# RalphAS/PeriodicSchurDecompositions.jl

Hardware: AMD Instinct MI355X
Metric: PSD sweeps/sec (pschur! n=1024 p=64 Float64, Hessenberg+Q+iteration, operands in HBM) (higher is better)
Workload: dtype f64

## Files before the change

### periodicschurdecompositions.jl_amd/csrc/psd_engine.cpp

```cpp
#include <atomic>
#include "psd_hess.h"
#include "psd_bhess.h"
#include "psd_hess2.h"
#include "psd_formq2.h"
#include "psd_real_qr.h"
#include "psd_apply2.h"
#include "psd_zhess.h"
#include "psd_zhess2.h"
#include "psd_zqz.h"
#include "psd_zord.h"
#include "psd_rord.h"
#include "psd_rgz.h"
#include "psd_zgz.h"
#include "psd_zgord.h"
#include "psd_grord.h"
#include "psd_rhessx.h"
#include "psd_check.h"
#include "psd_krylov.h"
#include "psd_evec.h"
#include "psd_gevec.h"
#include "psd_bevec.h"
#include "psd_zbevec.h"
#include "psd_bord.h"
#include "psd_zbqz.h"
// ... 190 lines not shown
        PSD_CHECK(psd_rt_malloc((void**)&tcnt, 2 * sizeof(int) * PSD_SLOTS * (size_t)(p + 8)));
        PSD_CHECK(psd_rt_malloc((void**)&ttr, 2 * sizeof(psd_tr) * PSD_SLOTS * (size_t)p * PSD_TR_CAP));
        PSD_CHECK(psd_rt_malloc((void**)&tgl, sizeof(psd_rglobal)));
        PSD_CHECK(psd_rt_malloc((void**)&tslotw, sizeof(int) * (8 * PSD_SLOTS + PSD_PLAN_INTS)));
        tcap_p = p;
        return 0;
    }
    void trelease() {
        if (tcst) psd_rt_free(tcst);
        if (tshift) psd_rt_free(tshift);
        if (tdesc) psd_rt_free(tdesc);
        if (tcnt) psd_rt_free(tcnt);
        if (ttr) psd_rt_free(ttr);
        if (tgl) psd_rt_free(tgl);
        if (tslotw) psd_rt_free(tslotw);
        tcst = nullptr; tshift = nullptr; tdesc = nullptr; tcnt = nullptr; ttr = nullptr;
        tgl = nullptr; tslotw = nullptr;
        tcap_p = 0;
    }
    double* fqT = nullptr;
    size_t fqT_doubles = 0;
    int formq_blocked = 1;
#ifndef PSD_HOSTSIM
    hipGraphExec_t hess_exec = nullptr;
    int hess_graph_n = 0, hess_graph_p = 0;
    double* h2ring = nullptr;
    int h2ring_n = 0;
    double* zh2ring = nullptr;
    int zh2ring_n = 0;
    std::vector<hipEvent_t> h2ev;
    int hess_async = -1;
    int hess_lookahead = 1;
    int hess_xcd = 1;
    int hess_fit = 15;
#endif
    int shard_rank = 0, shard_world = 1;
    int batch_group = 0;
    int bh_nmax = PSD_BH_NMAX;
    int zb_nmax = PSD_ZB_NMAX;
    int bev_nmax = PSD_BEV_NMAX;
    int bord_nmax = PSD_BORD_NMAX;
    int bord_w = 0;
    void slice(int p, int& lo, int& hi) const {
        const int base = p / shard_world, rem = p % shard_world;
        lo = shard_rank * base + (shard_rank < rem ? shard_rank : rem);
        hi = lo + base + (shard_rank < rem ? 1 : 0);
    }
    int train_stop = 1;
    int train_wdiv = 0;
    int train_long = 256;
    int band_helper = 1;
    int zstream = 3;
    int zcdefer = 0;
    int redge = 0, cedge = 0;
    int rdefer = 1;
    int cdefer = 1;
    int overlap = 3;
    int far_grid = 0;
    bool counted = false;
    bool pipe_ok = false;
#ifndef PSD_HOSTSIM
    hipStream_t stream2 = nullptr;
    hipStream_t stream3 = nullptr;
    hipStream_t stream4 = nullptr;
    int hess_pipe_depth = 3;
    int hess_pipe = 1;
// ... 341 lines not shown
};
#endif

namespace {

void fill_bytes(psd_stats* s, int n, int p, int wantT, int wantZ, const std::vector<int>& log) {
    if (!s) return;
    double b = 0.0;
    const double E = 8.0;
    for (size_t q = 0; q + 2 < log.size(); q += 3) {
        if (log[q] != 0) continue;
        const double w = log[q + 2] - log[q + 1] + 1;
        if (!wantT) b += 2 * E * p * w * w + (wantZ ? 2 * E * p * w * n : 0.0);
        else b += 2 * E * p * w * (wantZ ? (2.0 * n + 1) : (n + 1.0));
    }
    s->bytes_sweeps = b;
}

static inline bool psd_pipe_form(const psd_ctx* c) {
#ifndef PSD_HOSTSIM
    if (!c->stream4 || c->hess_pipe == 0) return false;
    return c->hess_pipe == 2 || c->shard_world > 1 || c->pipe_ok;
#else
    (void)c;
    return false;
#endif
}

#ifndef PSD_HOSTSIM

struct h2_diag {
    psd_ctx* c;
    long long* t = nullptr;
    static constexpr size_t words = 1024 * 8 + 1024 * 4;
    h2_diag(psd_ctx* c_, psd_hess2_args& ha) : c(c_) {
        ha.fault = -1;
        if (const char* e = psd_env_diag("PSD_H2_FAULT")) ha.fault = atoi(e);
        ha.trace = nullptr;
        ha.trace_hi = 0x7fffffff;
        const char* e = psd_env_diag("PSD_H2_TRACE");
        if (!e) return;
        if (atoi(e) > 1) ha.trace_hi = atoi(e);
        if (psd_rt_malloc((void**)&t, words * sizeof(long long)) != 0) t = nullptr;
        else if (psd_rt_memset(t, 0, words * sizeof(long long), c->stream) == 0) ha.trace = t;
    }
    ~h2_diag() {
        if (!t) return;
        std::vector<long long> h(words);
        (void)psd_rt_sync(c->stream);
        (void)hipMemcpy(h.data(), t, sizeof(long long) * h.size(), hipMemcpyDeviceToHost);
        double acc[8] = {0};
        int cnt = 0;
        double per = 0;
        for (int q = 1; q < 1023; ++q) {
            const long long* a = &h[(size_t)q * 8];
            const long long* pr = &h[(size_t)(q - 1) * 8];
            if (a[0] == 0 || a[6] == 0 || pr[0] == 0 || a[0] < pr[0]) continue;
            for (int k = 1; k <= 6; ++k) acc[k] += (double)(a[k] - a[k - 1]);
            per += (double)(a[0] - pr[0]);
            ++cnt;
        }
        if (cnt) fprintf(stderr, "psd hess2 trace (last %d links, block 2, us): link period %.2f | ring loads %.2f | norm reduce %.2f | larfg %.2f | v to LDS + publish %.2f | gemv %.2f | finish %.2f\n", cnt, per / cnt / 100.0, acc[1] / cnt / 100.0, acc[2] / cnt / 100.0, acc[3] / cnt / 100.0, acc[4] / cnt / 100.0, acc[5] / cnt / 100.0, acc[6] / cnt / 100.0);
        const long long* bk = &h[1024 * 8];
        long long t0 = 0;
        for (int q = 0; q < 1024; ++q)
            if (bk[4 * q] && (!t0 || bk[4 * q] < t0)) t0 = bk[4 * q];
        if (t0) {
            fprintf(stderr, "psd hess2 trace, one link, per block (start, end in us after the first start):");
            for (int q = 0; q < 1024; ++q)
                if (bk[4 * q] && (q < 12 || q % 16 == 0)) fprintf(stderr, " b%d %.2f-%.2f", q, (bk[4 * q] - t0) / 100.0, (bk[4 * q + 1] - t0) / 100.0);
            double lastend = 0, maxstart = 0;
            for (int q = 0; q < 1024; ++q)
                if (bk[4 * q]) {
                    if ((bk[4 * q + 1] - t0) / 100.0 > lastend) lastend = (bk[4 * q + 1] - t0) / 100.0;
                    if ((bk[4 * q] - t0) / 100.0 > maxstart) maxstart = (bk[4 * q] - t0) / 100.0;
                }
            fprintf(stderr, " | last start %.2f last end %.2f\n", maxstart, lastend);
        }
        psd_rt_free(t);
    }
};
struct h2_no_diag {
    h2_no_diag(psd_ctx*, psd_zhess2_args&) {}
};

template <typename T> struct h2_type;
template <> struct h2_type<double> {
    typedef psd_hess2_args args;
    typedef h2_diag diag;
    static constexpr int NT = PSD_H2_NT, ROWS = PSD_H2_ROWS;
    static constexpr int CR_LARGE = 8;
    static constexpr int PIPE_NMAX = 2048;
    static constexpr bool FIT = true;
    template <int NKB> static constexpr int CPW = (NKB <= 16) ? 4 : 1;
    template <int NK, int CR>
    static void link(int grid, size_t lds, hipStream_t s, const args& ha, int n, int i, int j, int nC, int nT) {
        hipLaunchKernelGGL((psd_hess2_link<NK, CR>), dim3(grid), dim3(NT), lds, s, ha, n, i, j, nC, nT);
    }
    template <int NK, int CPW_>
    static void bulk(int gridx, int K, size_t lds, hipStream_t s, const args& ha, int n, int idx0, int nT) {
        hipLaunchKernelGGL((psd_hess2_bulk<NK, CPW_>), dim3(gridx, K), dim3(NT), lds, s, ha, n, idx0, nT);
    }
    static double*& ring(psd_ctx* c) { return c->h2ring; }
    static int& ring_n(psd_ctx* c) { return c->h2ring_n; }
    static size_t slot_doubles(int n) { return psd_h2_slot_doubles(n); }
    static int pipe(const psd_ctx* c, int n, args& ha) {
        ha.pipe = 2;
        if (n > 512 && n <= 1024) ha.xcd = 0;
        return (c->hess_pipe_depth >= 3 && c->stream2 && n <= 1024) ? 3 : 2;
    }
};
template <> struct h2_type<psd_z> {
    typedef psd_zhess2_args args;
    typedef h2_no_diag diag;
    static constexpr int NT = PSD_ZH2_NT, ROWS = PSD_ZH2_ROWS;
    static constexpr int CR_LARGE = 4;
    static constexpr int PIPE_NMAX = 1024;
    static constexpr bool FIT = false;
    template <int NKB> static constexpr int CPW = 1;
    template <int NK, int CR>
    static void link(int grid, size_t lds, hipStream_t s, const args& ha, int n, int i, int j, int nC, int nT) {
        hipLaunchKernelGGL((psd_zhess2_link<NK, CR>), dim3(grid), dim3(NT), lds, s, ha, n, i, j, nC, nT);
    }
    template <int NK, int>
    static void bulk(int gridx, int K, size_t lds, hipStream_t s, const args& ha, int n, int idx0, int nT) {
        hipLaunchKernelGGL((psd_zhess2_bulk<NK>), dim3(gridx, K), dim3(NT), lds, s, ha, n, idx0, nT);
    }
    static double*& ring(psd_ctx* c) { return c->zh2ring; }
    static int& ring_n(psd_ctx* c) { return c->zh2ring_n; }
    static size_t slot_doubles(int n) { return psd_zh2_slot_doubles(n); }
    static int pipe(const psd_ctx*, int, args& ha) {
        ha.pipe = 1;
        return 2;
    }
};

template <typename T> size_t h2_lds(int n) { return ((size_t)n + 8 + 2 * h2_type<T>::NT + 64) * sizeof(T); }
template <typename T, int CR> struct h2_grid {
    static constexpr int RPL = 128 / (int)sizeof(T), G = 8 * RPL / CR;
    int nC, nT;
    h2_grid(int n, int xcd) {
        const int nc = (n + CR - 1) / CR;
        nC = ((xcd && CR < RPL) ? (nc + G - 1) / G * G : nc) + 1;
        nT = (n + h2_type<T>::ROWS - 1) / h2_type<T>::ROWS;
    }
};

template <typename T, int NKB, int CR> struct h2_launcher {
    typedef h2_type<T> Tr;
    typedef typename Tr::args args;
    static constexpr int CPW = Tr::template CPW<NKB>;
    const h2_grid<T, CR> g;
    const size_t lds;
    const int n, p, GS;
    const int fit;
    const args& ha;
    h2_launcher(psd_ctx* c, int n_, int p_, const args& ha_)
        : g(n_, ha_.xcd), lds(h2_lds<T>(n_)), n(n_), p(p_), GS((ha_.xcd && CR < g.RPL) ? g.RPL / CR : 0), fit(Tr::FIT ? c->hess_fit : 0), ha(ha_) {}
    void link(hipStream_t s, int i, int j, bool fused) const {
        psd_h2_geom q{NKB, g.nC, fused ? g.nT : 0, fused ? (n + 3) / 4 : 0};
        if constexpr (Tr::FIT) {
            if (fit) {
                const psd_h2_geom f = psd_h2_fit_chain(n, p, (i - 1) * p + (p - j), CR, GS, fused);
                if (fit & 1) q.nC = f.nC;
                if (fit & 2) q.NK = f.NK;
                if (fit & 4) q.nT = f.nT, q.nB = f.nB;
                const int grid = q.nC + q.nT + q.nB;
                switch (q.NK) {
                    case 4: if constexpr (NKB > 4) return Tr::template link<4, CR>(grid, lds, s, ha, n, i, j, q.nC, q.nT); break;
                    case 8: if constexpr (NKB > 8) return Tr::template link<8, CR>(grid, lds, s, ha, n, i, j, q.nC, q.nT); break;
                    case 16: if constexpr (NKB > 16) return Tr::template link<16, CR>(grid, lds, s, ha, n, i, j, q.nC, q.nT); break;
                    default: break;
                }
            }
        }
        Tr::template link<NKB, CR>(q.nC + q.nT + q.nB, lds, s, ha, n, i, j, q.nC, q.nT);
    }
    void bulk(hipStream_t s, int idx0, int K) const {
        psd_h2_geom q{NKB, 0, g.nT, (n + 3) / 4};
        if constexpr (Tr::FIT) {
            if (fit) {
                psd_h2_geom f = q;
                psd_h2_fit_panel(n, p, idx0, K, 4 * CPW, f);
                if (fit & 4) q.nT = f.nT, q.nB = f.nB;
                if (fit & 8) q.NK = f.NK;
                const int gx = q.nT + q.nB > 0 ? q.nT + q.nB : 1;
                switch (q.NK) {
                    case 4: if constexpr (NKB > 4) return Tr::template bulk<4, CPW>(gx, K, lds, s, ha, n, idx0, q.nT); break;
                    case 8: if constexpr (NKB > 8) return Tr::template bulk<8, CPW>(gx, K, lds, s, ha, n, idx0, q.nT); break;
                    case 16: if constexpr (NKB > 16) return Tr::template bulk<16, CPW>(gx, K, lds, s, ha, n, idx0, q.nT); break;
                    default: break;
                }
            }
        }
        Tr::template bulk<NKB, CPW>(q.nT + q.nB > 0 ? q.nT + q.nB : 1, K, lds, s, ha, n, idx0, q.nT);
    }
};

constexpr size_t PSD_H2_EVENTS = 34;
int h2_events(psd_ctx* c) {
    std::vector<hipEvent_t> made;
    for (size_t q = c->h2ev.size(); q < PSD_H2_EVENTS; ++q) {
        hipEvent_t e = nullptr;
        const int rc = (int)hipEventCreateWithFlags(&e, hipEventDisableTiming);
        if (rc != 0) {
            for (hipEvent_t m : made) (void)hipEventDestroy(m);
            return PSD_INFO_RUNTIME + (rc & 0xffff);
        }
        made.push_back(e);
// ... 62 lines not shown
        PSD_CHECK(hipStreamWaitEvent(c->stream, evJ, 0));
    }
    PSD_CHECK(hipStreamWaitEvent(c->stream, evB[(nbatch - 1) & 7], 0));
    return 0;
}

template <typename T, int NK, int CR>
int h2_form(psd_ctx* c, int n, int p, const typename h2_type<T>::args& ha, int K, int NS) {
    return NS ? h2_chain<T, NK, CR>(c, n, p, ha, K, NS) : h2_launches<T, NK, CR>(c, n, p, ha);
}

template <typename T>
int hessenberg2_dev(psd_ctx* c, int n, int p, T* dH, T* dtau) {
    typedef h2_type<T> Tr;
    if (h2_lds<T>(n) > 64 * 1024) return PSD_INFO_NOTIMPL;
    const size_t slot = Tr::slot_doubles(n);
    const size_t ringbytes = PSD_H2_RING * slot * sizeof(double) + 64;
    double*& ring = Tr::ring(c);
    if (!ring || Tr::ring_n(c) < n) {
        if (ring) psd_rt_free(ring);
        ring = nullptr;
        PSD_CHECK(psd_rt_malloc((void**)&ring, ringbytes));
        Tr::ring_n(c) = n;
    }
    PSD_CHECK(psd_rt_memset(ring, 0, ringbytes, c->stream));
    typename Tr::args ha{};
    ha.H = dH;
    ha.tau = dtau;
    ha.ring = ring;
    ha.p = p;
    ha.ringmask = 3;
    ha.xcd = c->hess_xcd;
    ha.err = (int*)(ring + PSD_H2_RING * slot);
    typename Tr::diag diag(c, ha);
    int K = c->hess_async;
    if (K < 0) K = (p >= 32 && n >= 512) ? ((p >= 48 && c->hess_pipe && c->stream4 && n <= Tr::PIPE_NMAX) ? 24 : 16) : 0;
    if (K > 0 && p >= 9 * K) K = (p + 7) / 8;
    int NS = 0;
    if (K > 0 && p >= 2 * K && p + K + 2 <= PSD_H2_RING && c->stream3) {
        ha.ringmask = PSD_H2_RING - 1;
        NS = (n <= Tr::PIPE_NMAX && psd_pipe_form(c)) ? Tr::pipe(c, n, ha) : 1;
    }
    int rc;
    if (n <= 256) rc = h2_form<T, 4, 8>(c, n, p, ha, K, NS);
    else if (n <= 512) rc = h2_form<T, 8, 8>(c, n, p, ha, K, NS);
    else if (n <= 1024) rc = NS >= 2 ? h2_form<T, 16, 8>(c, n, p, ha, K, NS) : h2_form<T, 16, 4>(c, n, p, ha, K, NS);
    else rc = h2_form<T, 32, Tr::CR_LARGE>(c, n, p, ha, K, NS);
    if (rc != 0 || NS < 2) return rc;
    int herr = 0;
    PSD_CHECK(psd_rt_d2h(&herr, ha.err, sizeof(int), c->stream));
    PSD_CHECK(psd_rt_sync(c->stream));
    return herr ? PSD_INFO_RUNTIME + 0xfffb : 0;
}
#endif

int hessenberg_dev(psd_ctx* c, int n, int p, double* dH, double* dtau) {
    PSD_CHECK(psd_rt_memset(dtau, 0, sizeof(double) * (size_t)n * p, c->stream));
    const size_t lds_refl = PSD_HESS_NT * 8;
    const size_t lds_apply = (PSD_HESS_NT + (size_t)n + 8) * 8;
    if (n < 2) return 0;
#ifndef PSD_HOSTSIM
    if (p >= 3 && n <= 2048 && c->hess_lookahead) return hessenberg2_dev(c, n, p, dH, dtau);
#endif
    if (!c->hargs) PSD_CHECK(psd_rt_malloc((void**)&c->hargs, sizeof(psd_hess_args)));
    psd_hess_args ha;
    ha.H = dH;
    ha.tau = dtau;
// ... 634 lines not shown
        c->ncu = ncu;
        int keep = PSD_SLOTS;
        if (const char* e = psd_env_diag("PSD_OVERLAP_CUS")) keep = atoi(e);
        hipError_t rc = hipErrorInvalidValue;
        if (c->overlap && ncu > keep + 32 && keep > 0 && ncu <= 1024) {
            uint32_t mask[32];
            memset(mask, 0, sizeof(mask));
            for (int q = keep; q < ncu; ++q) mask[q >> 5] |= (1u << (q & 31));
            rc = hipExtStreamCreateWithCUMask(&c->stream2, (uint32_t)((ncu + 31) / 32), mask);
            if (rc == hipSuccess) c->far_grid = (ncu - keep) * 8;
        }
        if (rc != hipSuccess) rc = hipStreamCreate(&c->stream2);
        if (rc != hipSuccess) {
            psd_destroy(c);
            return PSD_INFO_RUNTIME + 4;
        }
        int keeph = 64;
        if (const char* e = psd_env_diag("PSD_HESS_CUS")) keeph = atoi(e);
        rc = hipErrorInvalidValue;
        if (ncu > keeph + 32 && keeph > 0 && ncu <= 1024) {
            uint32_t mask[32];
            memset(mask, 0, sizeof(mask));
            for (int q = keeph; q < ncu; ++q) mask[q >> 5] |= (1u << (q & 31));
            rc = hipExtStreamCreateWithCUMask(&c->stream3, (uint32_t)((ncu + 31) / 32), mask);
        }
        if (rc != hipSuccess) rc = hipStreamCreate(&c->stream3);
        if (rc != hipSuccess) {
            psd_destroy(c);
            return PSD_INFO_RUNTIME + 4;
        }
        if (hipStreamCreate(&c->stream4) != hipSuccess) c->stream4 = nullptr;
        if (const char* e = psd_env("PSD_H2_PIPE")) c->hess_pipe = atoi(e);
        if (const char* e = psd_env("PSD_H2_DEPTH")) c->hess_pipe_depth = atoi(e);
        if (const char* e = psd_env("PSD_H2_FIT")) c->hess_fit = atoi(e);
    }
#endif
#ifndef PSD_HOSTSIM
    if (const char* e = psd_env("PSD_HESS_LOOKAHEAD")) c->hess_lookahead = atoi(e);
    if (const char* e = psd_env("PSD_HESS_ASYNC")) c->hess_async = atoi(e);
#endif
#ifdef PSD_HOSTSIM
    if (const char* e = psd_env("PSD_OVERLAP")) c->overlap = atoi(e);
#endif
    if (const char* e = psd_env("PSD_CDEFER")) c->cdefer = atoi(e);
    if (const char* e = psd_env("PSD_RDEFER")) c->rdefer = atoi(e);
    if (const char* e = psd_env("PSD_ZCDEFER")) c->zcdefer = atoi(e);
    if (const char* e = psd_env("PSD_ZSTREAM")) c->zstream = atoi(e);
    if (const char* e = psd_env("PSD_RDEFER_EDGE")) c->redge = atoi(e);
    if (const char* e = psd_env("PSD_CDEFER_EDGE")) c->cedge = atoi(e);
    if (const char* e = psd_env("PSD_ORD_PIPE")) c->ord_pipe = atoi(e);
    if (const char* e = psd_env("PSD_FORMQ_BLOCKED")) c->formq_blocked = atoi(e);
    if (const char* e = psd_env("PSD_BATCH_GROUP")) c->batch_group = atoi(e) > 0 ? atoi(e) : 0;
    if (const char* e = psd_env_diag("PSD_BH_NMAX")) c->bh_nmax = (atoi(e) >= 1 && atoi(e) <= 2048) ? atoi(e) : PSD_BH_NMAX;
    if (const char* e = psd_env_diag("PSD_ZB_NMAX")) c->zb_nmax = (atoi(e) >= 1 && atoi(e) <= 2048) ? atoi(e) : PSD_ZB_NMAX;
    if (const char* e = psd_env_diag("PSD_BEV_NMAX")) c->bev_nmax = (atoi(e) >= 1 && atoi(e) <= 2048) ? atoi(e) : PSD_BEV_NMAX;
    if (const char* e = psd_env("PSD_BORD_NMAX")) c->bord_nmax = (atoi(e) >= 1 && atoi(e) < PSD_BORD_NMAX) ? atoi(e) : PSD_BORD_NMAX;
    if (const char* e = psd_env("PSD_BORD_W")) c->bord_w = (atoi(e) >= 1 && atoi(e) <= 32) ? atoi(e) : 0;
    if (const char* e = psd_env("PSD_BAND_HELPER")) c->band_helper = atoi(e);
    if (const char* e = psd_env_diag("PSD_TRAIN_LONG")) c->train_long = atoi(e);
    if (const char* e = psd_env_diag("PSD_TRAIN_STOP")) c->train_stop = atoi(e);
    if (const char* e = psd_env_diag("PSD_TRAIN_WDIV")) c->train_wdiv = atoi(e) > 0 ? atoi(e) : 0;
    if (const char* e = psd_env("PSD_MB")) c->mblock = atoi(e);
    if (const char* e = psd_env_diag("PSD_TRAIN_MB")) c->train_mb_m = atoi(e);
    if (const char* e = psd_env_diag("PSD_APPLY_WL")) c->apply_worklist = atoi(e);
    if (const char* e = psd_env_diag("PSD_APPLY_WL_GRID")) c->apply_wl_grid = atoi(e) > 0 ? atoi(e) : 2048;
    if (const char* e = psd_env_diag("PSD_APPLY_WL2")) c->apply_wl2 = atoi(e);
// ... 2089 lines not shown
```

### periodicschurdecompositions.jl_amd/csrc/psd_hess2.h

```cpp
#pragma once
#include "psd_scalar.h"

#define PSD_H2_ROWS 8

#ifndef PSD_HOSTSIM
#define PSD_H2_NT 256
#define PSD_H2_RING 256

#define PSD_H2_WAIT_TICKS 300000000LL
__device__ __forceinline__ bool psd_h2_wait_expired(int& spins, long long& t0) {
    if ((++spins & 255) != 0) return false;
    const long long now = (long long)__builtin_amdgcn_s_memrealtime();
    if (t0 == 0) {
        t0 = now;
        return false;
    }
    return now - t0 > PSD_H2_WAIT_TICKS;
}

struct psd_hess2_args {
    double* H;
    double* tau;
    double* ring;
    int p;
    int ringmask;
    int xcd;
    long long* trace;
    int trace_hi;
    int pipe;
    int* err;
    int fault;
};
PSD_HD size_t psd_h2_slot_doubles(int n) { return 5 * (size_t)(n + 8) + 8 + 2 * (size_t)(n / 4 + 2); }
struct psd_h2_slot {
    double *v, *w, *col, *hdr, *part;
    unsigned long long* rec;
};
PSD_HD unsigned long long psd_h2_tag(int slot) { return ((unsigned long long)(unsigned)(slot + 3)) * 0x9E3779B97F4A7C15ull | 1ull; }
PSD_D psd_h2_slot psd_h2_get(const psd_hess2_args* G, int n, int q) {
    double* b = G->ring + (size_t)(q & G->ringmask) * psd_h2_slot_doubles(n);
    psd_h2_slot s;
    s.v = b;
    s.w = b + (n + 8);
    s.col = b + 2 * (size_t)(n + 8);
    s.hdr = b + 3 * (size_t)(n + 8);
    s.part = s.hdr + 8;
    s.rec = (unsigned long long*)(s.part + 2 * (size_t)(n / 4 + 2));
    return s;
}
struct psd_h2_link {
    int valid, i, j, r0;
};
PSD_D psd_h2_link psd_h2_linkat(int i, int j, int d, int n, int p) {
    int jj = j - d, ii = i;
    if (jj < 1) {
        jj += p;
        ii += 1;
    } else if (jj > p) {
        jj -= p;
        ii -= 1;
    }
    psd_h2_link L;
    L.valid = (ii >= 1 && ii <= n - 1) ? 1 : 0;
    L.i = ii;
// ... 73 lines not shown
    double acc = 1.0;
    if (fabs(beta) < sfmin) {
        const double rsfmin = 1.0 / sfmin;
        bool smallb = true;
        while (smallb) {
            kount += 1;
            acc *= rsfmin;
            beta *= rsfmin;
            alpha *= rsfmin;
            smallb = (fabs(beta) < sfmin) && (kount < 20);
        }
        xnorm *= acc;
        beta = -copysign(hypot(alpha, xnorm), alpha);
    }
    tau = (beta - alpha) / beta;
    mult = acc * (1.0 / (alpha - beta));
    for (int q = 0; q < kount; ++q) beta *= sfmin;
}

struct psd_h2_geom {
    int NK, nC, nT, nB;
};
PSD_HD int psd_h2_row0(int n, int p, int idx) {
    if (idx < 0) return 0;
    if (idx >= (n - 1) * p) return n;
    const int i = idx / p + 1, j = p - idx % p;
    return ((j == 1) ? i + 1 : i) - 1;
}
PSD_HD int psd_h2_fit_nk(int ext) {
    int nk = 4;
    while (64 * nk < ext) nk *= 2;
    return nk;
}
PSD_HD void psd_h2_fit_panel(int n, int p, int idx0, int K, int CPG, psd_h2_geom& g) {
    const int Q = (n - 1) * p;
    const int last = (idx0 + K - 1 < Q) ? idx0 + K - 1 : Q;
    const int ci = (idx0 < 0) ? 1 : ((idx0 >= Q) ? n : idx0 / p + 1);
    g.NK = psd_h2_fit_nk(n - psd_h2_row0(n, p, idx0 - 1));
    g.nT = (psd_h2_row0(n, p, last) + PSD_H2_ROWS - 1) / PSD_H2_ROWS;
    g.nB = (n - ci + CPG - 1) / CPG;
}
PSD_HD psd_h2_geom psd_h2_fit_chain(int n, int p, int q, int CR, int GS, bool fused) {
    psd_h2_geom g;
    g.NK = psd_h2_fit_nk(n - psd_h2_row0(n, p, q));
    g.nT = g.nB = 0;
    if (fused) psd_h2_fit_panel(n, p, q - 1, 1, 4, g);
    const int nc = (n + CR - 1) / CR, s0 = psd_h2_row0(n, p, q + 1) / CR;
    if (GS > 1) {
        const int nl = (nc + GS - 1) / GS - s0 / GS;
        g.nC = 1 + (nl + 7) / 8 * 8 * GS;
    } else {
        g.nC = 1 + (nc > s0 ? nc - s0 : 0);
    }
    return g;
}

#ifndef PSD_HOSTSIM

template <int NKC>
PSD_D void psd_h2_col_load(const double* M, int n, int R0, int mL, int c, int lane, double (&a0)[NKC], double (&a1)[NKC]) {
#pragma unroll
    for (int k = 0; k < NKC; ++k) {
        const int rr = 2 * lane + 128 * k;
        a0[k] = a1[k] = 0.0;
        if (rr < mL) psd_h2_ld2(M, n, R0 + rr, c, true, rr + 1 < mL, a0[k], a1[k]);
    }
// ... 133 lines not shown
#pragma unroll
    for (int k = 0; k < NKC; ++k) {
        const int rr = 2 * lane + 128 * k;
        a0[k] = a1[k] = 0.0;
        if (rr < mL) {
            const bool ok1 = rr + 1 < mL;
            psd_h2_ld2(M, n, R0 + rr, c, true, ok1, a0[k], a1[k]);
            if (vc != 0.0) {
                a0[k] -= vc * SR.w[R0 + rr];
                if (ok1) a1[k] -= vc * SR.w[R0 + rr + 1];
            }
            if (tauL != 0.0) {
                z += a0[k] * SL.v[rr];
                if (ok1) z += a1[k] * SL.v[rr + 1];
            }
        }
    }
    z = tauL * psd_h2_wave_sum(z);
#pragma unroll
    for (int k = 0; k < NKC; ++k) {
        const int rr = 2 * lane + 128 * k;
        if (rr < mL) {
            const bool ok1 = rr + 1 < mL;
            double x0 = a0[k], x1 = a1[k];
            if (tauL != 0.0) {
                x0 -= z * SL.v[rr];
                if (ok1) x1 -= z * SL.v[rr + 1];
            }
            psd_h2_st2(M, n, R0 + rr, c, true, ok1, x0, x1);
        }
    }
}

template <int NK, int CR>
__global__ void __launch_bounds__(PSD_H2_NT, ((NK > 16 || NK * CR > 128) ? ((NK * CR > 256) ? 1 : 2) : 4)) psd_hess2_link(const psd_hess2_args Gv, int n, int qi, int qj, int nC, int nT) {
    extern __shared__ __attribute__((aligned(16))) char psd_lds[];
    double* vs = (double*)psd_lds;
    double* red = vs + (n + 8);
    const psd_hess2_args* G = &Gv;
    const int p = G->p;
    const psd_h2_link L = psd_h2_linkat(qi, qj, 0, n, p);
    const int tid = threadIdx.x, lane = tid & 63, wave = tid >> 6;
    const int b = blockIdx.x;
    if (b < nC) {
        const psd_h2_link Ln = psd_h2_linkat(qi, qj, 1, n, p);
        if (!L.valid && !Ln.valid) return;
        if (!L.valid && qi > 1) return;
        const int q = L.valid ? 0 : -1;
        const int slot = qi * p - qj;
        long long* const trc = (G->trace != nullptr && b == 2 && tid == 0 && slot < G->trace_hi) ? (G->trace + (size_t)(slot & 1023) * 8) : nullptr;
#define PSD_H2_STAMP(i) do { if (trc) trc[i] = (long long)__builtin_amdgcn_s_memrealtime(); } while (0)
        PSD_H2_STAMP(0);
        long long* const blk = (G->trace != nullptr && tid == 0 && slot == G->trace_hi - 1 && b < 1024) ? (G->trace + 1024 * 8 + (size_t)b * 4) : nullptr;
        if (blk) {
            blk[0] = (long long)__builtin_amdgcn_s_memrealtime();
            blk[2] = (long long)__builtin_amdgcn_s_getreg(63492);
        }
        const psd_h2_slot S = psd_h2_get(G, n, slot), Sn = psd_h2_get(G, n, slot + 1);
        const int r0 = L.r0 - 1;
        const int m = (q >= 0) ? (n - r0) : 0;
        constexpr int RP = CR / 2;
        constexpr int CL = PSD_H2_NT / RP;
        constexpr int NKS = (64 * NK + CL - 1) / CL;
        const int ntileC = (n + CR - 1) / CR;
        const double* M = Ln.valid ? (G->H + (size_t)(Ln.j - 1) * n * n) : G->H;
        const int r0n = Ln.r0 - 1;
        const int cfirst = (q >= 0) ? r0 : (Ln.i - 1);
        int t = r0n / CR + (b - 1);
        if (G->xcd) {
            constexpr int GS = (CR < 16) ? 16 / CR : 1;
            const int idx = b - 1, grp0 = (r0n / CR) / GS;
            t = GS * (grp0 + (idx % 8) + 8 * (idx / (8 * GS))) + (idx / 8) % GS;
        }
        const bool strip = Ln.valid && b > 0 && t < ntileC && t >= r0n / CR;
        const int rp = tid % RP, cl = tid / RP;
        const int r = CR * t + 2 * rp;
        const bool ok0 = strip && r < n && r >= r0n, ok1 = strip && r + 1 < n && r + 1 >= r0n;
        constexpr int NK1 = (NKS + 1) / 2;
        double a0[NKS], a1[NKS];
        const int rfin = CR * t + tid;
        const bool fin = strip && tid < CR && rfin < n && rfin >= r0n;
        constexpr int NV = (64 * NK + PSD_H2_NT - 1) / PSD_H2_NT;
        double xcol[NV];
        double tau = 0.0, beta = 0.0, mult = 0.0, xnorm = 0.0;
        double am = 0.0, sq = 0.0, alpha = 0.0;
        const bool pipe = G->pipe != 0;
        if (q >= 0 && !pipe) {
            const int np_ = ntileC - r0 / CR;
            if (tid < np_) {
                am = S.part[2 * tid];
                sq = S.part[2 * tid + 1];
            }
            alpha = S.col[r0];
#pragma unroll
            for (int u = 0; u < NV; ++u) {
                const int k = tid + PSD_H2_NT * u;
                xcol[u] = (k < m) ? S.col[r0 + k] : 0.0;
            }
        }
        const double mfirst = fin ? M[(size_t)cfirst * n + rfin] : 0.0;
        if (q >= 0) {
#pragma unroll
            for (int k = 0; k < NKS; ++k) {
                const int cc = cl + CL * k;
                a0[k] = a1[k] = 0.0;
                if (cc < m) psd_h2_ld2(M, n, r, r0 + cc, ok0, ok1, a0[k], a1[k]);
            }
        }
        if (q >= 0 && pipe) {
            const unsigned long long tag = psd_h2_tag(slot);
            const unsigned long long* rec = S.rec + 2 * (size_t)r0;
            unsigned long long xb[NV], ab = 0;
            int spins = 0;
            long long wait_t0 = 0;
            if (G->pipe == 1) {
                const int rw = CR * (r0 / CR + tid);
                const int kw = (rw > r0) ? (rw - r0) : 0;
                const bool watch = kw < m && (tid == 0 || rw > r0);
                for (;;) {
                    bool okr = true;
                    if (watch) {
                        const unsigned long long x = __hip_atomic_load(rec + 2 * kw, __ATOMIC_RELAXED, __HIP_MEMORY_SCOPE_AGENT);
                        const unsigned long long cx = __hip_atomic_load(rec + 2 * kw + 1, __ATOMIC_RELAXED, __HIP_MEMORY_SCOPE_AGENT);
                        okr = (x ^ cx) == tag;
                    }
                    const bool giveup = __hip_atomic_load(G->err, __ATOMIC_RELAXED, __HIP_MEMORY_SCOPE_AGENT) != 0;
                    if (__syncthreads_and((okr || giveup) ? 1 : 0)) break;
                    if (psd_h2_wait_expired(spins, wait_t0)) {
                        if (tid == 0) __hip_atomic_store(G->err, 1, __ATOMIC_RELAXED, __HIP_MEMORY_SCOPE_AGENT);
                    }
                    __builtin_amdgcn_s_sleep(2);
                }
            }
            const __amdgpu_buffer_rsrc_t rsr = __builtin_amdgcn_make_buffer_rsrc((void*)rec, 0, m * 16, 0x00020000);
            for (;;) {
                bool okr = true;
#pragma unroll
                for (int u = 0; u < NV; ++u) {
                    const int k = tid + PSD_H2_NT * u;
                    xb[u] = 0;
                    if (PSD_H2_NT * u < m) {
                        const psd_h2_u4 t4 = __builtin_amdgcn_raw_buffer_load_b128(rsr, (k < m) ? (unsigned)k * 16u : 0xfffffff0u, 0, 16);
                        const unsigned long long x = ((unsigned long long)t4.y << 32) | t4.x, cx = ((unsigned long long)t4.w << 32) | t4.z;
                        okr = okr && (k >= m || (x ^ cx) == tag);
                        xb[u] = x;
                    }
                }
                asm volatile("" ::: "memory");
                const bool giveup = __hip_atomic_load(G->err, __ATOMIC_RELAXED, __HIP_MEMORY_SCOPE_AGENT) != 0;
                if (__syncthreads_and((okr || giveup) ? 1 : 0)) break;
                if (psd_h2_wait_expired(spins, wait_t0)) {
                    if (tid == 0) __hip_atomic_store(G->err, 1, __ATOMIC_RELAXED, __HIP_MEMORY_SCOPE_AGENT);
                }
                __builtin_amdgcn_s_sleep(2);
            }
            am = 0.0;
            sq = 0.0;
#pragma unroll
            for (int u = 0; u < NV; ++u) {
                const int k = tid + PSD_H2_NT * u;
                xcol[u] = (k < m) ? __longlong_as_double((long long)xb[u]) : 0.0;
                if (k >= 1 && k < m) {
                    am = fmax(am, fabs(xcol[u]));
                    sq = __builtin_fma(xcol[u], xcol[u], sq);
                }
                if (k < m) vs[k] = (k == 0) ? 0.0 : xcol[u];
            }
            (void)ab;
        }
        if (q >= 0) {
            PSD_H2_STAMP(1);
            if (pipe) {
                const double amw = psd_h2_wave_max(am);
                const double s2w = psd_h2_wave_sum(sq);
                if (lane == 0) {
                    red[2 * wave] = amw;
                    red[2 * wave + 1] = s2w;
                }
                if (tid == 0) red[8] = xcol[0];
                __syncthreads();
                alpha = red[8];
                const double amax = fmax(fmax(red[0], red[2]), fmax(red[4], red[6]));
                const double s2 = (red[1] + red[3]) + (red[5] + red[7]);
                if (m > 1 && amax > 0.0) {
                    if (amax < 1e140 && amax > 1e-140) {
                        double g, rg;
                        psd_sqrt_pair_fast(s2, g, rg);
                        xnorm = g;
                    } else {
                        __syncthreads();
                        double ss = 0.0;
#pragma unroll
                        for (int u = 0; u < NV; ++u) {
                            const int k = tid + PSD_H2_NT * u;
                            if (k >= 1 && k < m) {
                                const double z = xcol[u] / amax;
                                ss += z * z;
                            }
                        }
                        ss = psd_h2_wave_sum(ss);
                        if (lane == 0) red[16 + wave] = ss;
                        __syncthreads();
                        xnorm = amax * sqrt((red[16] + red[17]) + (red[18] + red[19]));
                    }
                }
            } else {
                const double amw = psd_h2_wave_max(am);
                double ssw = 0.0;
                if (amw > 0.0) {
                    const double f = am / amw;
                    ssw = sq * (f * f);
                }
                ssw = psd_h2_wave_sum(ssw);
                if (lane == 0) {
                    red[2 * wave] = amw;
                    red[2 * wave + 1] = ssw;
                }
                __syncthreads();
                const double amax = fmax(fmax(red[0], red[2]), fmax(red[4], red[6]));
                double tot = 0.0;
                if (amax > 0.0) {
#pragma unroll
                    for (int wv = 0; wv < 4; ++wv) {
                        const double f = red[2 * wv] / amax;
                        tot += red[2 * wv + 1] * (f * f);
                    }
                }
                xnorm = (m > 1) ? amax * sqrt(tot) : 0.0;
            }
            PSD_H2_STAMP(2);
            if (!pipe || b == 0) psd_h2_larfg(alpha, xnorm, tau, beta, mult);
            PSD_H2_STAMP(3);
            if (!pipe) {
#pragma unroll
                for (int u = 0; u < NV; ++u) {
                    const int k = tid + PSD_H2_NT * u;
                    if (k < m) vs[k] = (k == 0) ? 1.0 : xcol[u] * mult;
                }
                __syncthreads();
            }
            if (b == 0) {
                double* Mq = G->H + (size_t)(L.j - 1) * n * n;
                const int c = L.i - 1;
#pragma unroll
                for (int u = 0; u < NV; ++u) {
                    const int k = tid + PSD_H2_NT * u;
                    if (k < m) {
                        const double vk = (k == 0) ? 1.0 : xcol[u] * mult;
                        S.v[k] = vk;
                        Mq[(size_t)c * n + r0 + k] = (tau != 0.0) ? ((k == 0) ? beta : vk) : xcol[u];
                    }
                }
                if (tid == 0) {
                    S.hdr[0] = tau;
                    S.hdr[1] = beta;
                    G->tau[(size_t)(L.j - 1) * n + (L.i - 1)] = tau;
                }
            }
        }
        if (!strip) return;
        PSD_H2_STAMP(4);
        double acc0 = 0.0, acc1 = 0.0;
        if (q >= 0 && (pipe || tau != 0.0)) {
#pragma unroll
            for (int k = 0; k < NKS; ++k) {
                const int cc = cl + CL * k;
                if (cc < m) {
                    const double vv = vs[cc];
                    acc0 += a0[k] * vv;
                    acc1 += a1[k] * vv;
                }
            }
        }
        double* const redg = pipe ? (red + 64) : red;
#pragma unroll
        for (int sft = RP; sft < 64; sft <<= 1) {
            acc0 += __shfl_xor(acc0, sft, 64);
            acc1 += __shfl_xor(acc1, sft, 64);
        }
        if (lane < RP) {
            redg[(wave * RP + lane) * 2] = acc0;
            redg[(wave * RP + lane) * 2 + 1] = acc1;
        }
        if (pipe && q >= 0) psd_h2_larfg(alpha, xnorm, tau, beta, mult);
        __syncthreads();
        PSD_H2_STAMP(5);
        double amt = 0.0, y = 0.0;
        if (fin) {
            double w = redg[tid] + redg[CR + tid] + redg[2 * CR + tid] + redg[3 * CR + tid];
            if (pipe && q >= 0) w = (tau != 0.0) ? __builtin_fma(mult, w, mfirst) : 0.0;
            y = mfirst - tau * w;
            if (pipe) {
                const unsigned long long yb = (unsigned long long)__double_as_longlong(y);
                __hip_atomic_store(Sn.rec + 2 * (size_t)rfin, yb, __ATOMIC_RELAXED, __HIP_MEMORY_SCOPE_AGENT);
                __hip_atomic_store(Sn.rec + 2 * (size_t)rfin + 1, yb ^ psd_h2_tag(slot + 1) ^ ((G->fault == slot + 1) ? 0x10ull : 0ull), __ATOMIC_RELAXED,
                                   __HIP_MEMORY_SCOPE_AGENT);
            } else {
                Sn.col[rfin] = y;
            }
            S.w[rfin] = w;
            if (rfin > r0n) amt = fabs(y);
            else y = 0.0;
        }
        if (wave == 0 && !pipe) {
            const double amax = psd_h2_wave_max(amt);
            double sq = 0.0;
            if (amax > 0.0 && amt > 0.0) {
                const double z = y / amax;
                sq = z * z;
            }
            sq = psd_h2_wave_sum(sq);
            if (lane == 0) {
                Sn.part[2 * (t - r0n / CR)] = amax;
                Sn.part[2 * (t - r0n / CR) + 1] = sq;
            }
        }
        PSD_H2_STAMP(6);
        if (blk) blk[1] = (long long)__builtin_amdgcn_s_memrealtime();
        return;
    }
    psd_h2_bulk_body<NK>(G, n, psd_h2_linkat(qi, qj, -1, n, p), psd_h2_linkat(qi, qj, -2, n, p), qi * p - qj - 1, b - nC, nT, vs, red);
}

template <int NK, int CPW = (NK <= 16 ? 4 : 1)>
__global__ void __launch_bounds__(PSD_H2_NT, (NK > 16 ? 2 : (CPW > 1 ? 3 : 4))) psd_hess2_bulk(const psd_hess2_args Gv, int n, int idx0, int nT) {
    extern __shared__ __attribute__((aligned(16))) char psd_lds[];
    double* vs = (double*)psd_lds;
    double* red = vs + (n + 8);
    const int p = Gv.p;
    const int idx = idx0 + (int)blockIdx.y;
    const int Q = (n - 1) * p;
    if (idx > Q) return;
    psd_h2_link Lb, La;
    Lb.i = idx / p + 1;
    Lb.j = p - idx % p;
    Lb.valid = (idx < Q) ? 1 : 0;
    Lb.r0 = (Lb.j == 1) ? (Lb.i + 1) : Lb.i;
    La = psd_h2_linkat(Lb.i, Lb.j, -1, n, p);
    psd_h2_bulk_body<NK, CPW>(&Gv, n, Lb, La, idx, (int)blockIdx.x, nT, vs, red);
}

#endif
```

Before: 2570.

## Add multi-strip workgroups, skip re-polling valid ring entries, optional backoff wait

```diff
diff --git a/periodicschurdecompositions.jl_amd/csrc/psd_engine.cpp b/periodicschurdecompositions.jl_amd/csrc/psd_engine.cpp
--- a/periodicschurdecompositions.jl_amd/csrc/psd_engine.cpp
+++ b/periodicschurdecompositions.jl_amd/csrc/psd_engine.cpp
@@ -246,6 +246,9 @@
     int hess_async = -1;
     int hess_lookahead = 1;
     int hess_xcd = 1;
+    int hess_spw = 0;
+    int hess_skipv = 1;
+    int hess_backoff = 0;
     int hess_fit = 15;
 #endif
     int shard_rank = 0, shard_world = 1;
@@ -653,8 +656,9 @@
 struct h2_diag {
     psd_ctx* c;
     long long* t = nullptr;
-    static constexpr size_t words = 1024 * 8 + 1024 * 4;
-    h2_diag(psd_ctx* c_, psd_hess2_args& ha) : c(c_) {
+    size_t len = 1024;
+    size_t words() const { return len * 8 + 1024 * 4; }
+    h2_diag(psd_ctx* c_, psd_hess2_args& ha, int n) : c(c_) {
         ha.fault = -1;
         if (const char* e = psd_env_diag("PSD_H2_FAULT")) ha.fault = atoi(e);
         ha.trace = nullptr;
@@ -662,27 +666,47 @@
         const char* e = psd_env_diag("PSD_H2_TRACE");
         if (!e) return;
         if (atoi(e) > 1) ha.trace_hi = atoi(e);
-        if (psd_rt_malloc((void**)&t, words * sizeof(long long)) != 0) t = nullptr;
-        else if (psd_rt_memset(t, 0, words * sizeof(long long), c->stream) == 0) ha.trace = t;
+        while (len < (size_t)(n - 1) * ha.p && len < (1u << 17)) len *= 2;
+        ha.trace_mask = (int)len - 1;
+        if (psd_rt_malloc((void**)&t, words() * sizeof(long long)) != 0) t = nullptr;
+        else if (psd_rt_memset(t, 0, words() * sizeof(long long), c->stream) == 0) ha.trace = t;
     }
     ~h2_diag() {
         if (!t) return;
-        std::vector<long long> h(words);
+        std::vector<long long> h(words());
         (void)psd_rt_sync(c->stream);
         (void)hipMemcpy(h.data(), t, sizeof(long long) * h.size(), hipMemcpyDeviceToHost);
         double acc[8] = {0};
         int cnt = 0;
         double per = 0;
-        for (int q = 1; q < 1023; ++q) {
-            const long long* a = &h[(size_t)q * 8];
-            const long long* pr = &h[(size_t)(q - 1) * 8];
+        for (size_t q = 1; q + 1 < len; ++q) {
+            const long long* a = &h[q * 8];
+            const long long* pr = &h[(q - 1) * 8];
             if (a[0] == 0 || a[6] == 0 || pr[0] == 0 || a[0] < pr[0]) continue;
             for (int k = 1; k <= 6; ++k) acc[k] += (double)(a[k] - a[k - 1]);
             per += (double)(a[0] - pr[0]);
             ++cnt;
         }
-        if (cnt) fprintf(stderr, "psd hess2 trace (last %d links, block 2, us): link period %.2f | ring loads %.2f | norm reduce %.2f | larfg %.2f | v to LDS + publish %.2f | gemv %.2f | finish %.2f\n", cnt, per / cnt / 100.0, acc[1] / cnt / 100.0, acc[2] / cnt / 100.0, acc[3] / cnt / 100.0, acc[4] / cnt / 100.0, acc[5] / cnt / 100.0, acc[6] / cnt / 100.0);
-        const long long* bk = &h[1024 * 8];
+        if (cnt) fprintf(stderr, "psd hess2 trace (%d links, block 2, us): link period %.2f | ring loads %.2f | norm reduce %.2f | larfg %.2f | v to LDS + publish %.2f | gemv %.2f | finish %.2f\n", cnt, per / cnt / 100.0, acc[1] / cnt / 100.0, acc[2] / cnt / 100.0, acc[3] / cnt / 100.0, acc[4] / cnt / 100.0, acc[5] / cnt / 100.0, acc[6] / cnt / 100.0);
+        size_t last = 0;
+        for (size_t q = 0; q + 1 < len; ++q)
+            if (h[q * 8 + 1] && h[q * 8 + 6]) last = q + 1;
+        for (int part = 0; last >= 8 && part < 4; ++part) {
+            double per4 = 0, wait4 = 0, rounds4 = 0;
+            int cnt4 = 0;
+            const size_t lo = part * last / 4, hi = (part + 1) * last / 4;
+            for (size_t q = lo; q < hi; ++q) {
+                const long long* a = &h[q * 8];
+                const long long* nx = &h[(q + 1) * 8];
+                if (a[1] == 0 || a[6] == 0 || nx[6] <= a[6]) continue;
+                per4 += (double)(nx[6] - a[6]);
+                wait4 += (double)(a[1] - a[0]);
+                rounds4 += (double)a[7];
+                ++cnt4;
+            }
+            if (cnt4) fprintf(stderr, "psd hess2 trace, links %zu-%zu (%d recorded): link period %.2f us | wait %.2f us | failed poll rounds %.1f\n", lo, hi - 1, cnt4, per4 / cnt4 / 100.0, wait4 / cnt4 / 100.0, rounds4 / cnt4);
+        }
+        const long long* bk = &h[len * 8];
         long long t0 = 0;
         for (int q = 0; q < 1024; ++q)
             if (bk[4 * q] && (!t0 || bk[4 * q] < t0)) t0 = bk[4 * q];
@@ -702,7 +726,7 @@
     }
 };
 struct h2_no_diag {
-    h2_no_diag(psd_ctx*, psd_zhess2_args&) {}
+    h2_no_diag(psd_ctx*, psd_zhess2_args&, int) {}
 };
 
 template <typename T> struct h2_type;
@@ -713,10 +737,11 @@
     static constexpr int CR_LARGE = 8;
     static constexpr int PIPE_NMAX = 2048;
     static constexpr bool FIT = true;
+    static constexpr bool SPW = true;
     template <int NKB> static constexpr int CPW = (NKB <= 16) ? 4 : 1;
-    template <int NK, int CR>
+    template <int NK, int CR, int SPW_ = 1>
     static void link(int grid, size_t lds, hipStream_t s, const args& ha, int n, int i, int j, int nC, int nT) {
-        hipLaunchKernelGGL((psd_hess2_link<NK, CR>), dim3(grid), dim3(NT), lds, s, ha, n, i, j, nC, nT);
+        hipLaunchKernelGGL((psd_hess2_link<NK, CR, SPW_>), dim3(grid), dim3(NT * SPW_), lds, s, ha, n, i, j, nC, nT);
     }
     template <int NK, int CPW_>
     static void bulk(int gridx, int K, size_t lds, hipStream_t s, const args& ha, int n, int idx0, int nT) {
@@ -726,9 +751,12 @@
     static int& ring_n(psd_ctx* c) { return c->h2ring_n; }
     static size_t slot_doubles(int n) { return psd_h2_slot_doubles(n); }
     static int pipe(const psd_ctx* c, int n, args& ha) {
+        const int NS = (c->hess_pipe_depth >= 3 && c->stream2 && n <= 1024) ? 3 : 2;
+        ha.skipv = c->hess_skipv ? 1 : 0;
+        ha.backoff = (NS == 3 && c->hess_backoff) ? 1 : 0;
         ha.pipe = 2;
         if (n > 512 && n <= 1024) ha.xcd = 0;
-        return (c->hess_pipe_depth >= 3 && c->stream2 && n <= 1024) ? 3 : 2;
+        return NS;
     }
 };
 template <> struct h2_type<psd_z> {
@@ -738,8 +766,9 @@
     static constexpr int CR_LARGE = 4;
     static constexpr int PIPE_NMAX = 1024;
     static constexpr bool FIT = false;
+    static constexpr bool SPW = false;
     template <int NKB> static constexpr int CPW = 1;
-    template <int NK, int CR>
+    template <int NK, int CR, int = 1>
     static void link(int grid, size_t lds, hipStream_t s, const args& ha, int n, int i, int j, int nC, int nT) {
         hipLaunchKernelGGL((psd_zhess2_link<NK, CR>), dim3(grid), dim3(NT), lds, s, ha, n, i, j, nC, nT);
     }
@@ -756,7 +785,7 @@
     }
 };
 
-template <typename T> size_t h2_lds(int n) { return ((size_t)n + 8 + 2 * h2_type<T>::NT + 64) * sizeof(T); }
+template <typename T> size_t h2_lds(int n, int nt = h2_type<T>::NT) { return ((size_t)n + 8 + 2 * nt + 64) * sizeof(T); }
 template <typename T, int CR> struct h2_grid {
     static constexpr int RPL = 128 / (int)sizeof(T), G = 8 * RPL / CR;
     int nC, nT;
@@ -775,27 +804,41 @@
     const size_t lds;
     const int n, p, GS;
     const int fit;
+    const int spw;
     const args& ha;
     h2_launcher(psd_ctx* c, int n_, int p_, const args& ha_)
-        : g(n_, ha_.xcd), lds(h2_lds<T>(n_)), n(n_), p(p_), GS((ha_.xcd && CR < g.RPL) ? g.RPL / CR : 0), fit(Tr::FIT ? c->hess_fit : 0), ha(ha_) {}
+        : g(n_, ha_.xcd), lds(h2_lds<T>(n_)), n(n_), p(p_), GS((ha_.xcd && CR < g.RPL) ? g.RPL / CR : 0), fit(Tr::FIT ? c->hess_fit : 0), spw(c->hess_spw), ha(ha_) {}
+    template <int NK_> void link_nk(int SPW, int grid, hipStream_t s, int i, int j, int nC, int nT) const {
+        if constexpr (Tr::SPW && CR == Tr::ROWS && NK_ <= 16) {
+            if (SPW == 2) return Tr::template link<NK_, CR, 2>(grid, h2_lds<T>(n, 2 * Tr::NT), s, ha, n, i, j, nC, nT);
+            if (SPW == 4) return Tr::template link<NK_, CR, 4>(grid, h2_lds<T>(n, 4 * Tr::NT), s, ha, n, i, j, nC, nT);
+        }
+        Tr::template link<NK_, CR, 1>(grid, lds, s, ha, n, i, j, nC, nT);
+    }
     void link(hipStream_t s, int i, int j, bool fused) const {
         psd_h2_geom q{NKB, g.nC, fused ? g.nT : 0, fused ? (n + 3) / 4 : 0};
+        const int idx = (i - 1) * p + (p - j);
+        int SPW = 1;
+        if constexpr (Tr::SPW && CR == Tr::ROWS && NKB <= 16) {
+            if (!fused && ha.pipe == 2) SPW = spw ? spw : psd_h2_fit_spw(n - psd_h2_row0(n, p, idx));
+            if (SPW > 1) q.nC = (n + CR * SPW - 1) / (CR * SPW) + 1;
+        }
         if constexpr (Tr::FIT) {
             if (fit) {
-                const psd_h2_geom f = psd_h2_fit_chain(n, p, (i - 1) * p + (p - j), CR, GS, fused);
+                const psd_h2_geom f = psd_h2_fit_chain(n, p, idx, CR * SPW, SPW > 1 ? 0 : GS, fused);
                 if (fit & 1) q.nC = f.nC;
                 if (fit & 2) q.NK = f.NK;
                 if (fit & 4) q.nT = f.nT, q.nB = f.nB;
                 const int grid = q.nC + q.nT + q.nB;
                 switch (q.NK) {
-                    case 4: if constexpr (NKB > 4) return Tr::template link<4, CR>(grid, lds, s, ha, n, i, j, q.nC, q.nT); break;
-                    case 8: if constexpr (NKB > 8) return Tr::template link<8, CR>(grid, lds, s, ha, n, i, j, q.nC, q.nT); break;
-                    case 16: if constexpr (NKB > 16) return Tr::template link<16, CR>(grid, lds, s, ha, n, i, j, q.nC, q.nT); break;
+                    case 4: if constexpr (NKB > 4) return link_nk<4>(SPW, grid, s, i, j, q.nC, q.nT); break;
+                    case 8: if constexpr (NKB > 8) return link_nk<8>(SPW, grid, s, i, j, q.nC, q.nT); break;
+                    case 16: if constexpr (NKB > 16) return link_nk<16>(SPW, grid, s, i, j, q.nC, q.nT); break;
                     default: break;
                 }
             }
         }
-        Tr::template link<NKB, CR>(q.nC + q.nT + q.nB, lds, s, ha, n, i, j, q.nC, q.nT);
+        link_nk<NKB>(SPW, q.nC + q.nT + q.nB, s, i, j, q.nC, q.nT);
     }
     void bulk(hipStream_t s, int idx0, int K) const {
         psd_h2_geom q{NKB, 0, g.nT, (n + 3) / 4};
@@ -924,7 +967,7 @@
     ha.ringmask = 3;
     ha.xcd = c->hess_xcd;
     ha.err = (int*)(ring + PSD_H2_RING * slot);
-    typename Tr::diag diag(c, ha);
+    typename Tr::diag diag(c, ha, n);
     int K = c->hess_async;
     if (K < 0) K = (p >= 32 && n >= 512) ? ((p >= 48 && c->hess_pipe && c->stream4 && n <= Tr::PIPE_NMAX) ? 24 : 16) : 0;
     if (K > 0 && p >= 9 * K) K = (p + 7) / 8;
@@ -1625,6 +1668,9 @@
         if (hipStreamCreate(&c->stream4) != hipSuccess) c->stream4 = nullptr;
         if (const char* e = psd_env("PSD_H2_PIPE")) c->hess_pipe = atoi(e);
         if (const char* e = psd_env("PSD_H2_DEPTH")) c->hess_pipe_depth = atoi(e);
+        if (const char* e = psd_env("PSD_H2_SPW")) c->hess_spw = (atoi(e) == 1 || atoi(e) == 2 || atoi(e) == 4) ? atoi(e) : 0;
+        if (const char* e = psd_env("PSD_H2_BACKOFF")) c->hess_backoff = atoi(e);
+        if (const char* e = psd_env("PSD_H2_SKIPV")) c->hess_skipv = atoi(e);
         if (const char* e = psd_env("PSD_H2_FIT")) c->hess_fit = atoi(e);
     }
 #endif
diff --git a/periodicschurdecompositions.jl_amd/csrc/psd_hess2.h b/periodicschurdecompositions.jl_amd/csrc/psd_hess2.h
--- a/periodicschurdecompositions.jl_amd/csrc/psd_hess2.h
+++ b/periodicschurdecompositions.jl_amd/csrc/psd_hess2.h
@@ -26,10 +26,13 @@
     int ringmask;
     int xcd;
     long long* trace;
+    int trace_mask;
     int trace_hi;
     int pipe;
     int* err;
     int fault;
+    int skipv;
+    int backoff;
 };
 PSD_HD size_t psd_h2_slot_doubles(int n) { return 5 * (size_t)(n + 8) + 8 + 2 * (size_t)(n / 4 + 2); }
 struct psd_h2_slot {
@@ -169,6 +172,7 @@
     while (64 * nk < ext) nk *= 2;
     return nk;
 }
+PSD_HD int psd_h2_fit_spw(int ) { return 1; }
 PSD_HD void psd_h2_fit_panel(int n, int p, int idx0, int K, int CPG, psd_h2_geom& g) {
     const int Q = (n - 1) * p;
     const int last = (idx0 + K - 1 < Q) ? idx0 + K - 1 : Q;
@@ -368,15 +372,18 @@
     }
 }
 
-template <int NK, int CR>
-__global__ void __launch_bounds__(PSD_H2_NT, ((NK > 16 || NK * CR > 128) ? ((NK * CR > 256) ? 1 : 2) : 4)) psd_hess2_link(const psd_hess2_args Gv, int n, int qi, int qj, int nC, int nT) {
+template <int NK, int CR, int SPW = 1>
+__global__ void __launch_bounds__(PSD_H2_NT * SPW, ((NK > 16 || NK * CR > 128) ? ((NK * CR > 256) ? 1 : 2) : 4 / SPW)) psd_hess2_link(const psd_hess2_args Gv, int n, int qi, int qj, int nC, int nT) {
+    static_assert(SPW == 1 || ((SPW == 2 || SPW == 4) && CR == PSD_H2_ROWS && NK <= 16), "several strips per workgroup: 8-row strips of the four-to-a-CU kernels only");
     extern __shared__ __attribute__((aligned(16))) char psd_lds[];
     double* vs = (double*)psd_lds;
     double* red = vs + (n + 8);
     const psd_hess2_args* G = &Gv;
     const int p = G->p;
     const psd_h2_link L = psd_h2_linkat(qi, qj, 0, n, p);
-    const int tid = threadIdx.x, lane = tid & 63, wave = tid >> 6;
+    const int grp = (SPW > 1) ? (int)(threadIdx.x >> 8) : 0;
+    const int tid = (SPW > 1) ? (int)(threadIdx.x & 255) : (int)threadIdx.x, lane = tid & 63, wave = tid >> 6;
+    const bool g0 = (SPW == 1) || grp == 0;
     const int b = blockIdx.x;
     if (b < nC) {
         const psd_h2_link Ln = psd_h2_linkat(qi, qj, 1, n, p);
@@ -384,10 +391,10 @@
         if (!L.valid && qi > 1) return;
         const int q = L.valid ? 0 : -1;
         const int slot = qi * p - qj;
-        long long* const trc = (G->trace != nullptr && b == 2 && tid == 0 && slot < G->trace_hi) ? (G->trace + (size_t)(slot & 1023) * 8) : nullptr;
+        long long* const trc = (G->trace != nullptr && b == 2 && threadIdx.x == 0 && slot < G->trace_hi) ? (G->trace + (size_t)(slot & G->trace_mask) * 8) : nullptr;
 #define PSD_H2_STAMP(i) do { if (trc) trc[i] = (long long)__builtin_amdgcn_s_memrealtime(); } while (0)
         PSD_H2_STAMP(0);
-        long long* const blk = (G->trace != nullptr && tid == 0 && slot == G->trace_hi - 1 && b < 1024) ? (G->trace + 1024 * 8 + (size_t)b * 4) : nullptr;
+        long long* const blk = (G->trace != nullptr && threadIdx.x == 0 && slot == G->trace_hi - 1 && b < 1024) ? (G->trace + (size_t)(G->trace_mask + 1) * 8 + (size_t)b * 4) : nullptr;
         if (blk) {
             blk[0] = (long long)__builtin_amdgcn_s_memrealtime();
             blk[2] = (long long)__builtin_amdgcn_s_getreg(63492);
@@ -402,8 +409,8 @@
         const double* M = Ln.valid ? (G->H + (size_t)(Ln.j - 1) * n * n) : G->H;
         const int r0n = Ln.r0 - 1;
         const int cfirst = (q >= 0) ? r0 : (Ln.i - 1);
-        int t = r0n / CR + (b - 1);
-        if (G->xcd) {
+        int t = (SPW > 1) ? SPW * (r0n / (CR * SPW) + (b - 1)) + grp : r0n / CR + (b - 1);
+        if (SPW == 1 && G->xcd) {
             constexpr int GS = (CR < 16) ? 16 / CR : 1;
             const int idx = b - 1, grp0 = (r0n / CR) / GS;
             t = GS * (grp0 + (idx % 8) + 8 * (idx / (8 * GS))) + (idx / 8) % GS;
@@ -420,7 +427,7 @@
         double xcol[NV];
         double tau = 0.0, beta = 0.0, mult = 0.0, xnorm = 0.0;
         double am = 0.0, sq = 0.0, alpha = 0.0;
-        const bool pipe = G->pipe != 0;
+        const bool pipe = SPW > 1 || G->pipe != 0;
         if (q >= 0 && !pipe) {
             const int np_ = ntileC - r0 / CR;
             if (tid < np_) {
@@ -447,9 +454,9 @@
             const unsigned long long tag = psd_h2_tag(slot);
             const unsigned long long* rec = S.rec + 2 * (size_t)r0;
             unsigned long long xb[NV], ab = 0;
-            int spins = 0;
+            int spins = 0, rounds = 0;
             long long wait_t0 = 0;
-            if (G->pipe == 1) {
+            if (SPW == 1 && G->pipe == 1) {
                 const int rw = CR * (r0 / CR + tid);
                 const int kw = (rw > r0) ? (rw - r0) : 0;
                 const bool watch = kw < m && (tid == 0 || rw > r0);
@@ -468,25 +475,57 @@
                     __builtin_amdgcn_s_sleep(2);
                 }
             }
+            if (G->backoff) {
+                const psd_h2_link Lp = psd_h2_linkat(qi, qj, -1, n, p);
+                if (Lp.valid) {
+                    const unsigned long long* recp = psd_h2_get(G, n, slot - 1).rec + 2 * (size_t)(Lp.r0 - 1);
+                    const unsigned long long tagp = psd_h2_tag(slot - 1);
+                    for (;;) {
+                        bool okr = true;
+                        if (threadIdx.x == 0) {
+                            const unsigned long long x = __hip_atomic_load(recp, __ATOMIC_RELAXED, __HIP_MEMORY_SCOPE_AGENT);
+                            const unsigned long long cx = __hip_atomic_load(recp + 1, __ATOMIC_RELAXED, __HIP_MEMORY_SCOPE_AGENT);
+                            okr = (x ^ cx) == tagp || __hip_atomic_load(G->err, __ATOMIC_RELAXED, __HIP_MEMORY_SCOPE_AGENT) != 0;
+                        }
+                        if (__syncthreads_and(okr ? 1 : 0)) break;
+                        if (psd_h2_wait_expired(spins, wait_t0)) {
+                            if (threadIdx.x == 0) __hip_atomic_store(G->err, 1, __ATOMIC_RELAXED, __HIP_MEMORY_SCOPE_AGENT);
+                        }
+                        __builtin_amdgcn_s_sleep(32);
+                    }
+                }
+            }
             const __amdgpu_buffer_rsrc_t rsr = __builtin_amdgcn_make_buffer_rsrc((void*)rec, 0, m * 16, 0x00020000);
+            bool have[NV];
+            psd_h2_u4 t4[NV];
+#pragma unroll
+            for (int u = 0; u < NV; ++u) {
+                have[u] = false;
+                t4[u] = psd_h2_u4{0u, 0u, 0u, 0u};
+            }
+            const bool skipv = G->skipv != 0;
             for (;;) {
                 bool okr = true;
 #pragma unroll
                 for (int u = 0; u < NV; ++u) {
                     const int k = tid + PSD_H2_NT * u;
-                    xb[u] = 0;
-                    if (PSD_H2_NT * u < m) {
-                        const psd_h2_u4 t4 = __builtin_amdgcn_raw_buffer_load_b128(rsr, (k < m) ? (unsigned)k * 16u : 0xfffffff0u, 0, 16);
-                        const unsigned long long x = ((unsigned long long)t4.y << 32) | t4.x, cx = ((unsigned long long)t4.w << 32) | t4.z;
-                        okr = okr && (k >= m || (x ^ cx) == tag);
-                        xb[u] = x;
+                    if (g0 && PSD_H2_NT * u < m && !have[u]) t4[u] = __builtin_amdgcn_raw_buffer_load_b128(rsr, (k < m) ? (unsigned)k * 16u : 0xfffffff0u, 0, 16);
+                }
+#pragma unroll
+                for (int u = 0; u < NV; ++u) {
+                    const int k = tid + PSD_H2_NT * u;
+                    if (g0 && PSD_H2_NT * u < m && !have[u]) {
+                        const bool v = k >= m || ((t4[u].x ^ t4[u].z) == (unsigned)tag && (t4[u].y ^ t4[u].w) == (unsigned)(tag >> 32));
+                        okr = okr && v;
+                        have[u] = v && skipv;
                     }
                 }
                 asm volatile("" ::: "memory");
-                const bool giveup = __hip_atomic_load(G->err, __ATOMIC_RELAXED, __HIP_MEMORY_SCOPE_AGENT) != 0;
+                const bool giveup = g0 && __hip_atomic_load(G->err, __ATOMIC_RELAXED, __HIP_MEMORY_SCOPE_AGENT) != 0;
                 if (__syncthreads_and((okr || giveup) ? 1 : 0)) break;
+                ++rounds;
                 if (psd_h2_wait_expired(spins, wait_t0)) {
-                    if (tid == 0) __hip_atomic_store(G->err, 1, __ATOMIC_RELAXED, __HIP_MEMORY_SCOPE_AGENT);
+                    if (threadIdx.x == 0) __hip_atomic_store(G->err, 1, __ATOMIC_RELAXED, __HIP_MEMORY_SCOPE_AGENT);
                 }
                 __builtin_amdgcn_s_sleep(2);
             }
@@ -495,25 +534,27 @@
 #pragma unroll
             for (int u = 0; u < NV; ++u) {
                 const int k = tid + PSD_H2_NT * u;
+                xb[u] = ((unsigned long long)t4[u].y << 32) | t4[u].x;
                 xcol[u] = (k < m) ? __longlong_as_double((long long)xb[u]) : 0.0;
                 if (k >= 1 && k < m) {
                     am = fmax(am, fabs(xcol[u]));
                     sq = __builtin_fma(xcol[u], xcol[u], sq);
                 }
-                if (k < m) vs[k] = (k == 0) ? 0.0 : xcol[u];
+                if (g0 && k < m) vs[k] = (k == 0) ? 0.0 : xcol[u];
             }
             (void)ab;
+            if (trc) trc[7] = rounds;
         }
         if (q >= 0) {
             PSD_H2_STAMP(1);
             if (pipe) {
                 const double amw = psd_h2_wave_max(am);
                 const double s2w = psd_h2_wave_sum(sq);
-                if (lane == 0) {
+                if (g0 && lane == 0) {
                     red[2 * wave] = amw;
                     red[2 * wave + 1] = s2w;
                 }
-                if (tid == 0) red[8] = xcol[0];
+                if (g0 && tid == 0) red[8] = xcol[0];
                 __syncthreads();
                 alpha = red[8];
                 const double amax = fmax(fmax(red[0], red[2]), fmax(red[4], red[6]));
@@ -535,7 +576,7 @@
                             }
                         }
                         ss = psd_h2_wave_sum(ss);
-                        if (lane == 0) red[16 + wave] = ss;
+                        if (g0 && lane == 0) red[16 + wave] = ss;
                         __syncthreads();
                         xnorm = amax * sqrt((red[16] + red[17]) + (red[18] + red[19]));
                     }
@@ -575,7 +616,7 @@
                 }
                 __syncthreads();
             }
-            if (b == 0) {
+            if (b == 0 && g0) {
                 double* Mq = G->H + (size_t)(L.j - 1) * n * n;
                 const int c = L.i - 1;
 #pragma unroll
@@ -594,7 +635,7 @@
                 }
             }
         }
-        if (!strip) return;
+        if (SPW == 1 ? !strip : !(Ln.valid && b > 0 && SPW * (r0n / (CR * SPW) + (b - 1)) < ntileC)) return;
         PSD_H2_STAMP(4);
         double acc0 = 0.0, acc1 = 0.0;
         if (q >= 0 && (pipe || tau != 0.0)) {
@@ -608,7 +649,7 @@
                 }
             }
         }
-        double* const redg = pipe ? (red + 64) : red;
+        double* const redg = pipe ? (red + 64 + 4 * CR * grp) : red;
 #pragma unroll
         for (int sft = RP; sft < 64; sft <<= 1) {
             acc0 += __shfl_xor(acc0, sft, 64);
@@ -655,7 +696,8 @@
         if (blk) blk[1] = (long long)__builtin_amdgcn_s_memrealtime();
         return;
     }
-    psd_h2_bulk_body<NK>(G, n, psd_h2_linkat(qi, qj, -1, n, p), psd_h2_linkat(qi, qj, -2, n, p), qi * p - qj - 1, b - nC, nT, vs, red);
+    if constexpr (SPW == 1)
+        psd_h2_bulk_body<NK>(G, n, psd_h2_linkat(qi, qj, -1, n, p), psd_h2_linkat(qi, qj, -2, n, p), qi * p - qj - 1, b - nC, nT, vs, red);
 }
 
 template <int NK, int CPW = (NK <= 16 ? 4 : 1)>
```

Result: faster. 2642, median of 4 (+2.8%).
